# tum-vision/mem

Hardware: AMD Instinct MI355X
Metric: pretrain samples/sec (ViT-B, 224^2 event voxels) (higher is better)
Workload: dtype bf16

## Files before the change

### include/memhip.h

```cpp
#ifndef MEMHIP_H
#define MEMHIP_H

#include <stddef.h>
#include <stdint.h>

#ifdef __cplusplus
extern "C" {
#endif

#define MEMHIP_ABI_VERSION 10

#define MEMHIP_OK 0
#define MEMHIP_EINVAL (-1)
#define MEMHIP_EWORKSPACE (-2)
#define MEMHIP_ELAUNCH (-3)
#define MEMHIP_EUNSUPPORTED (-4)

typedef void* memhip_stream_t;

int memhip_abi_version(void);
const char* memhip_last_error(void);
const char* memhip_arch(void);
const char* memhip_build_flags(void);
int memhip_set_option(const char* name, int value);
// ... 238 lines not shown
  const int32_t* out_map;
  const memhip_dropout_t* dropout;
} memhip_branch_t;
typedef struct memhip_branch_bwd_args {
  const float* dx; int64_t lddx;
  int32_t M, D;
  memhip_branch_t branch;
} memhip_branch_bwd_args_t;
int memhip_branch_bwd(const memhip_branch_bwd_args_t* args, memhip_stream_t stream);
typedef struct memhip_ln_bwd_branch_args {
  const void* dy; int64_t lddy;
  const float* x; int64_t ldx;
  int32_t R, D;
  const float* gamma; const float* mean; const float* rstd;
  float* dres; int64_t lddres;
  float* dgamma; float* dbeta;
  const int32_t* in_map;
  memhip_branch_t branch;
} memhip_ln_bwd_branch_args_t;
int memhip_layernorm_bwd_branch(const memhip_ln_bwd_branch_args_t* args, memhip_stream_t stream);

int memhip_embed_bwd(const float* dx, int64_t lddx, const uint8_t* mask, int B, int L, int D,
                     void* dy_bf16, int64_t lddy, float* dcls, float* dmask_token, memhip_stream_t stream);

int memhip_cross_entropy(void* logits_bf16, int64_t ld, const int64_t* labels, int M, int V,
                         float grad_scale, float* row_loss, int32_t* row_correct, int write_grad,
                         float* out2, memhip_stream_t stream);

int memhip_attn_tokens_padded(int T);
int memhip_relpos_gather(const float* table, const int32_t* index , int T, int TP, int heads,
                         float* bias_pad, float* biasT_pad ,
                         memhip_stream_t stream);
int memhip_attn_fwd(const void* qkv, int64_t ldqkv, int B, int T, int D, int heads, const float* table,
                    int window_h, int window_w, void* out, int64_t ldo, float* lse, memhip_stream_t stream);
int memhip_attn_delta(const void* dout, const void* out, int64_t ldo, int64_t rows, int heads, float* delta,
                      memhip_stream_t stream);
typedef struct memhip_attn_bwd_args {
  const void* qkv; int64_t ldqkv;
  const void* dout; int64_t ldo;
  const void* out; int64_t ldout;
  const float* lse;
  float* delta;
  const float* table;
  int32_t window_h, window_w, B, T, D, heads;
  float scale;
  int32_t reserved0;
  void* dqkv; int64_t lddqkv;
  float* dtable; float* dq_bias; float* dv_bias;
  void* ws; int64_t ws_bytes;
} memhip_attn_bwd_args_t;
// ... 232 lines not shown
```

### mem_amd/csrc/rowops.hip

```cpp
#include "common.h"
#include "dropout.hpp"

#include <type_traits>

namespace {

using namespace memhip;

typedef __attribute__((ext_vector_type(4))) __bf16 bf16x4;
typedef __attribute__((ext_vector_type(8))) __bf16 bf16x8;

__device__ __forceinline__ float wsum(float v) {
  for (int o = 32; o > 0; o >>= 1) v += __shfl_xor(v, o);
  return v;
}
__device__ __forceinline__ float wmax(float v) {
  for (int o = 32; o > 0; o >>= 1) v = fmaxf(v, __shfl_xor(v, o));
  return v;
}

__device__ __forceinline__ float div_newton(float a, float b, float r) {
  const float q0 = a * r;
  return fmaf(fmaf(-q0, b, a), r, q0);
}

constexpr int kMaxChunks = 8;

template <bool FULL>
__device__ __forceinline__ bool chunk_ok(int i, int nch) {
  if constexpr (FULL) return true;
  else return i < nch;
}

// ... 601 lines not shown
        if (k < K) {
          const bf16x4 w = *reinterpret_cast<const bf16x4*>(wr + k);
          const float4 g = *reinterpret_cast<const float4*>(gr + k);
          s[c] += (float)w[0] * g.x + (float)w[1] * g.y + (float)w[2] * g.z + (float)w[3] * g.w;
        }
      }
    }
  }
#pragma unroll
  for (int c = 0; c < 4; ++c) {
    const float t = wsum(s[c]);
    if (lane == 0) red[wave][c] = t;
  }
  __syncthreads();
  if (threadIdx.x < 4 && n0 + (int)threadIdx.x < N) {
    const int n = n0 + threadIdx.x;
    float t = (red[0][threadIdx.x] + red[1][threadIdx.x]) + (red[2][threadIdx.x] + red[3][threadIdx.x]);
    if (b && db) t += b[n] * db[n];
    const float g = gamma[n];
    dgamma[n] = g != 0.f ? t / g : 0.f;
  }
}

__global__ __launch_bounds__(256) void embed_bwd_kernel(const float* __restrict__ dx, long long lddx,
                                                        const unsigned char* __restrict__ mask, int B,
                                                        int L, int D, __bf16* __restrict__ dy,
                                                        long long lddy, float* __restrict__ dcls,
                                                        float* __restrict__ dmask) {
  constexpr int U = 7;
  for (int c = threadIdx.x * 4; c < D; c += 256 * 4) {
    float4 cls{0, 0, 0, 0}, am{0, 0, 0, 0};
    for (int b = blockIdx.x; b < B; b += gridDim.x) {
      const float* row0 = dx + (long long)b * (L + 1) * lddx + c;
      const float4 dc = *reinterpret_cast<const float4*>(row0);
      cls.x += dc.x; cls.y += dc.y; cls.z += dc.z; cls.w += dc.w;
      const unsigned char* mk = mask + (long long)b * L;
      __bf16* out = dy + (long long)b * L * lddy + c;
      int p = 0;
      for (; p + U <= L; p += U) {
        float4 d[U];
#pragma unroll
        for (int u = 0; u < U; ++u) d[u] = *reinterpret_cast<const float4*>(row0 + (long long)(1 + p + u) * lddx);
#pragma unroll
        for (int u = 0; u < U; ++u) {
          const float w = (float)mk[p + u], q = 1.0f - w;
          am.x += d[u].x * w; am.y += d[u].y * w; am.z += d[u].z * w; am.w += d[u].w * w;
          bf16x4 o;
          o[0] = (__bf16)(d[u].x * q); o[1] = (__bf16)(d[u].y * q); o[2] = (__bf16)(d[u].z * q); o[3] = (__bf16)(d[u].w * q);
          *reinterpret_cast<bf16x4*>(out + (long long)(p + u) * lddy) = o;
        }
      }
      for (; p < L; ++p) {
        const float4 d = *reinterpret_cast<const float4*>(row0 + (long long)(1 + p) * lddx);
        const float w = (float)mk[p], q = 1.0f - w;
        am.x += d.x * w; am.y += d.y * w; am.z += d.z * w; am.w += d.w * w;
        bf16x4 o;
        o[0] = (__bf16)(d.x * q); o[1] = (__bf16)(d.y * q); o[2] = (__bf16)(d.z * q); o[3] = (__bf16)(d.w * q);
        *reinterpret_cast<bf16x4*>(out + (long long)p * lddy) = o;
      }
    }
    atomicAdd(dcls + c, cls.x); atomicAdd(dcls + c + 1, cls.y);
    atomicAdd(dcls + c + 2, cls.z); atomicAdd(dcls + c + 3, cls.w);
    atomicAdd(dmask + c, am.x); atomicAdd(dmask + c + 1, am.y);
    atomicAdd(dmask + c + 2, am.z); atomicAdd(dmask + c + 3, am.w);
  }
}

template <int VPT>
__global__ __launch_bounds__(256) void ce_kernel(__bf16* __restrict__ logits, long long ld,
                                                 const long long* __restrict__ labels, int V,
                                                 float grad_scale, float* __restrict__ row_loss,
                                                 int* __restrict__ row_correct, int write_grad) {
  __shared__ float sm[4];
  __shared__ int si[4];
  __shared__ float bc[2];
  const int r = blockIdx.x, tid = threadIdx.x, lane = tid & 63, wave = tid >> 6;
  bf16x8* row = reinterpret_cast<bf16x8*>(logits + (long long)r * ld);
  const int nch = V >> 3;
  float v[VPT][8];
  float mx = -INFINITY;
  int amax = 0x7fffffff;
#pragma unroll
  for (int c = 0; c < VPT; ++c) {
    const int i = tid + c * 256;
    if (i < nch) {
      const bf16x8 t = row[i];
#pragma unroll
// ... 57 lines not shown
        }
        row[i] = o;
      }
    }
  }
}

__global__ __launch_bounds__(256) void ce_reduce_kernel(const float* __restrict__ row_loss,
                                                        const int* __restrict__ row_correct, int M,
                                                        float* __restrict__ out) {
  __shared__ double sd[4];
  __shared__ int sc[4];
  double s = 0.0;
  int c = 0;
  for (int i = threadIdx.x; i < M; i += 256) { s += (double)row_loss[i]; c += row_correct[i]; }
  for (int o = 32; o > 0; o >>= 1) { s += __shfl_xor(s, o); c += __shfl_xor(c, o); }
  if ((threadIdx.x & 63) == 0) { sd[threadIdx.x >> 6] = s; sc[threadIdx.x >> 6] = c; }
  __syncthreads();
  if (threadIdx.x == 0) {
    const double t = (sd[0] + sd[1]) + (sd[2] + sd[3]);
    const int k = sc[0] + sc[1] + sc[2] + sc[3];
    out[0] = (float)(t / (double)M);
    out[1] = (float)k / (float)M;
  }
}

}

template <int MAXN, class F>
void dispatch_width(int D, F&& f) {
  const int nch = cdiv(D / 4, 64);
  const bool full = D % 256 == 0;
  const auto either = [&](auto N) { if (full) f(N, std::true_type{}); else f(N, std::false_type{}); };
  if (nch <= 1) either(std::integral_constant<int, 1>{});
  else if (nch <= 2) either(std::integral_constant<int, 2>{});
  else if (nch <= 3) either(std::integral_constant<int, 3>{});
  else if (MAXN == 4 || nch <= 4) either(std::integral_constant<int, 4>{});
  else if constexpr (MAXN == 8) {
    if (nch == 5 && full) f(std::integral_constant<int, 5>{}, std::true_type{});
    else if (nch == 8 && full) f(std::integral_constant<int, 8>{}, std::true_type{});
    else f(std::integral_constant<int, 8>{}, std::false_type{});
  }
}

extern "C" int memhip_layernorm_fwd(const float* x, int64_t ldx, const int32_t* row_idx, int R, int D,
                                    const float* gamma, const float* beta, float eps, void* y,
// ... 50 lines not shown
  if (M == 0) return MEMHIP_OK;
  MEMHIP_REQUIRE(args->dx && b.dy, "branch_bwd: null pointer");
  MEMHIP_REQUIRE(b.y || !b.dgamma, "branch_bwd: dgamma needs y (or use memhip_layerscale_grad)");
  MEMHIP_REQUIRE(args->lddx % 4 == 0 && b.ldy % 4 == 0 && b.lddy % 4 == 0, "branch_bwd: ld must be a multiple of 4");
  MEMHIP_REQUIRE(D <= 64 * 4 * kBrMaxChunks, "branch_bwd: D=%d too large", D);
  int grid = cdiv(M, 4);
  if (grid > 1024) grid = 1024;
  dispatch_width<kBrMaxChunks>(D, [&](auto N, auto F) {
    dispatch_bool(b.y, [&](auto Y) {
      if (b.dropout) branch_bwd_launch<decltype(N)::value, decltype(F)::value, decltype(Y)::value>(*args, grid, stream, drop_params(*b.dropout));
      else branch_bwd_launch<decltype(N)::value, decltype(F)::value, decltype(Y)::value>(*args, grid, stream);
      return 0;
    });
  });
  return check_launch("branch_bwd");
}

extern "C" int memhip_embed_bwd(const float* dx, int64_t lddx, const uint8_t* mask, int B, int L, int D,
                                void* dy, int64_t lddy, float* dcls, float* dmask_token,
                                memhip_stream_t stream) {
  MEMHIP_REQUIRE(B >= 0 && L > 0 && D > 0 && D % 4 == 0, "embed_bwd: bad shape");
  if (B == 0) return MEMHIP_OK;
  MEMHIP_REQUIRE(dx && mask && dy && dcls && dmask_token, "embed_bwd: null pointer");
  hipLaunchKernelGGL(embed_bwd_kernel, dim3(B < 128 ? B : 128), dim3(256), 0, as_stream(stream), dx, (long long)lddx, mask, B,
                     L, D, (__bf16*)dy, (long long)lddy, dcls, dmask_token);
  return check_launch("embed_bwd");
}

extern "C" int memhip_cross_entropy(void* logits, int64_t ld, const int64_t* labels, int M, int V,
                                    float grad_scale, float* row_loss, int32_t* row_correct,
                                    int write_grad, float* out2, memhip_stream_t stream) {
  MEMHIP_REQUIRE(M >= 0 && V > 0 && V % 8 == 0 && V <= 256 * 8 * 8, "cross_entropy: V=%d unsupported", V);
  if (M == 0) return MEMHIP_OK;
  MEMHIP_REQUIRE(logits && labels && row_loss && row_correct && out2, "cross_entropy: null pointer");
  MEMHIP_REQUIRE(ld % 8 == 0, "cross_entropy: ld must be a multiple of 8");
  hipStream_t s = as_stream(stream);
  const int nch = V / 8, vpt = cdiv(nch, 256);
  __bf16* lg = (__bf16*)logits;
  const long long* lab = (const long long*)labels;
#define CE_LAUNCH(N) hipLaunchKernelGGL(ce_kernel<N>, dim3(M), dim3(256), 0, s, lg, (long long)ld, lab, V, \
                                        grad_scale, row_loss, row_correct, write_grad)
  if (vpt <= 1) CE_LAUNCH(1);
  else if (vpt <= 2) CE_LAUNCH(2);
  else if (vpt <= 4) CE_LAUNCH(4);
  else CE_LAUNCH(8);
#undef CE_LAUNCH
  hipLaunchKernelGGL(ce_reduce_kernel, dim3(1), dim3(256), 0, s, row_loss, row_correct, M, out2);
  return check_launch("cross_entropy");
}

template <int NCH, bool FULL, bool HAS_Y, class... Drop>
static void ln_bwd_branch_launch(const memhip_ln_bwd_branch_args_t& a, int grid, memhip_stream_t stream, Drop... drop) {
  const memhip_branch_t& b = a.branch;
  hipLaunchKernelGGL((ln_bwd_branch_kernel<NCH, FULL, HAS_Y, Drop...>), dim3(grid), dim3(256), (size_t)16 * a.D * sizeof(float),
                     as_stream(stream), (const __bf16*)a.dy, (long long)a.lddy, a.x, (long long)a.ldx, a.R, a.D, a.gamma, a.mean,
                     a.rstd, a.dres, (long long)a.lddres, a.dgamma, a.dbeta, (const __bf16*)b.y, (long long)b.ldy, b.gamma,
                     b.rowmask, b.keep_prob, b.rows_per_sample > 0 ? b.rows_per_sample : 1, (__bf16*)b.dy, (long long)b.lddy,
                     b.dgamma, b.dbias, (const int*)a.in_map, (const int*)b.out_map, drop...);
}

extern "C" int memhip_layernorm_bwd_branch(const memhip_ln_bwd_branch_args_t* args, memhip_stream_t stream) {
  MEMHIP_REQUIRE(args, "layernorm_bwd_branch: null args");
  const memhip_ln_bwd_branch_args_t& a = *args;
  const memhip_branch_t& b = a.branch;
  const int R = a.R, D = a.D;
  MEMHIP_REQUIRE(R >= 0 && D > 0 && D % 4 == 0 && D <= 64 * 4 * 4, "layernorm_bwd_branch: D=%d unsupported (<= 1024)", D);
  MEMHIP_REQUIRE(!b.dropout || D % 8 == 0, "layernorm_bwd_branch_drop: D=%d must be a multiple of 8", D);
  MEMHIP_REQUIRE(!(a.in_map || b.out_map) || (!b.rowmask && !b.y && b.rows_per_sample > 0),
                 "layernorm_bwd_branch: sample maps exclude rowmask / y_branch");
  if (R == 0) return MEMHIP_OK;
  MEMHIP_REQUIRE(a.dy && a.x && a.gamma && a.mean && a.rstd && a.dres && a.dgamma && a.dbeta && b.dy,
// ... 34 lines not shown
```

### mem_amd/ops.py

```python
import ctypes as C

import torch

from ._lib import check, declare, f32, f64, i32, i64, lib, ptr, stream_ptr, sz, vp
from .vae_model import pack_convt_weight

EPI_BIAS_BF16, EPI_BIAS_GELU, EPI_RESIDUAL, EPI_DGELU, EPI_F32, EPI_PATCH_EMBED, EPI_BIAS_GELU_DG, EPI_MUL_AUX = range(8)
EPI_RESIDUAL_DROP = 8


class Dropout(C.Structure):
    _fields_ = [("key0", C.c_uint32), ("key1", C.c_uint32), ("site", C.c_uint32), ("thr", C.c_uint32), ("scale", f32),
                ("row0", i32)]


def dropout_params(key0, key1, site, p, row0=0):
    assert 0.0 <= p < 1.0, p
    return Dropout(int(key0) & 0xFFFFFFFF, int(key1) & 0xFFFFFFFF, int(site), int(round(p * 65536)), 1.0 / (1.0 - p), int(row0))


def with_row0(d, row0):
    return None if d is None else Dropout(d.key0, d.key1, d.site, d.thr, d.scale, int(row0))


# ... 260 lines not shown
        out = torch.empty((M,), dtype=torch.float32, device=logits.device)
    assert out.dtype == torch.float32 and out.numel() >= M
    check(lib.memhip_kl_uniform_rows(ptr(logits), _CONV_MODE[logits.dtype], logits.stride(0), M, N, ptr(out), stream_ptr()),
          "kl_uniform_rows")
    return out[:M]


def tok_flag_samples(gap, rms, B, hw, kappa, lst, count, stats=None):
    check(lib.memhip_tok_flag_samples(ptr(gap), ptr(rms), B, hw, float(kappa), ptr(lst), ptr(count), ptr(stats), stream_ptr()),
          "tok_flag_samples")


def tok_gather_images(x, mean, std, lst, count, offset, R, out, n_round):
    _, Cc, H, W = x.shape
    check(lib.memhip_tok_gather_images_f32(ptr(x), Cc, H, W, ptr(mean), ptr(std), ptr(lst), ptr(count), offset, R, ptr(out),
                                           ptr(n_round), stream_ptr()), "tok_gather_images_f32")


def tok_scatter_ids(ids_in, lst, n_round, offset, R, hw, ids_out):
    check(lib.memhip_tok_scatter_ids(ptr(ids_in), ptr(lst), ptr(n_round), offset, R, hw, ptr(ids_out), stream_ptr()),
          "tok_scatter_ids")


def embed_bwd(dx, mask_u8, B, L, D, dy, dcls, dmask_token):
    check(lib.memhip_embed_bwd(ptr(dx), dx.stride(0), ptr(mask_u8), B, L, D, ptr(dy), dy.stride(0), ptr(dcls),
                               ptr(dmask_token), stream_ptr()), "embed_bwd")


def cross_entropy(logits, labels, M, V, grad_scale, row_loss, row_correct, out2, write_grad=True):
    check(lib.memhip_cross_entropy(ptr(logits), logits.stride(0), ptr(labels), M, V, grad_scale, ptr(row_loss),
                                   ptr(row_correct), int(write_grad), ptr(out2), stream_ptr()), "cross_entropy")


def attn_tokens_padded(T):
    return lib.memhip_attn_tokens_padded(T)


def relpos_gather(table, index_i32, T, TP, heads, bias_pad, biasT_pad=None):
    check(lib.memhip_relpos_gather(ptr(table), ptr(index_i32), T, TP, heads, ptr(bias_pad), ptr(biasT_pad),
                                   stream_ptr()), "relpos_gather")


def attn_fwd(qkv, B, T, D, heads, table, window, out, lse):
    _timed(200, 4.0 * B * T * T * D, lambda: check(
        lib.memhip_attn_fwd(ptr(qkv), qkv.stride(0), B, T, D, heads, ptr(table), window[0], window[1], ptr(out),
                            out.stride(0), ptr(lse), stream_ptr()), "attn_fwd"))


def attn_delta(dout, out, rows, heads, delta):
    check(lib.memhip_attn_delta(ptr(dout), ptr(out), out.stride(0), rows, heads, ptr(delta), stream_ptr()),
          "attn_delta")


def attn_bwd_workspace(B, T, heads, window):
# ... 637 lines not shown
```

### mem_amd/vit_engine.py

```python
import math
from collections import namedtuple

import torch

from . import ops

ALIGN = 1024

Branch = namedtuple("Branch", "n rows gemm_rows ridx smap cmap rowmask keep_prob")


def _pad(n, a):
    return (n + a - 1) // a * a


def flat_layout(shapes, skip, order, aliases=()):
    decays = lambda n: not (len(shapes[n]) == 1 or n.endswith(".bias") or n in skip)
    segs, buckets, flags, off = {}, [], [], 0
    for bname, entries in order:
        b0 = off
        for e in entries:
            if isinstance(e, tuple):
                (n, k), flag = e, 0
            elif e in shapes:
# ... 197 lines not shown
        ops.zero_(self.flat_g[o:o + _pad(k, ALIGN)])

    def set_gelu_dg(self, on):
        self.epi_gelu, self.epi_dgelu = (ops.EPI_BIAS_GELU_DG, ops.EPI_MUL_AUX) if on else (ops.EPI_BIAS_GELU, ops.EPI_DGELU)

    def ensure_batch(self, B, Mm_max, keep=True):
        if B > self.B:
            self._alloc_forward(B)
        if keep and self.B_stash < self.B:
            self._alloc_stash()
        if Mm_max > self.Mm_cap or (self.head_kind == "mlm" and not hasattr(self, "hN")):
            self._alloc_head(min(self.B * self.L, _pad(Mm_max + Mm_max // 16 + 1, 256)))

    def _alloc_head(self, Mm_cap):
        dev, bf, f32 = self.dev, torch.bfloat16, torch.float32
        D, V = self.D, self.V
        e = lambda *s, dt=bf: torch.empty(s, dtype=dt, device=dev)
        if self.head_kind == "mlm":
            self.hN = e(Mm_cap, D)
            self.meanN, self.rstdN = e(Mm_cap, dt=f32), e(Mm_cap, dt=f32)
            self.logits = e(Mm_cap, V)
            self.row_loss, self.row_ok = e(Mm_cap, dt=f32), torch.empty(Mm_cap, dtype=torch.int32, device=dev)
            self.dhN = e(Mm_cap, D)
            self.x_tail, self.dxc = e(max(Mm_cap, 1), D, dt=f32), e(max(Mm_cap, 1), D, dt=f32)
            self.y_tail = torch.zeros((_pad(max(Mm_cap, 1), 256), D), dtype=bf, device=dev)
        self.Mm_cap = Mm_cap

    def _act_set(self, B):
        dev, bf, f32 = self.dev, torch.bfloat16, torch.float32
        D, Hd, M = self.D, self.hidden, B * self.T
        Ma = M + 256
        e = lambda *s, dt=bf: torch.empty(s, dtype=dt, device=dev)
        z = lambda *s, dt=bf: torch.zeros(s, dtype=dt, device=dev)
        return dict(h1=z(Ma, D), qkv=z(Ma, 3 * D), ao=z(Ma, D), h2=z(Ma, D), hpre=z(Ma, Hd),
                    a=z(Ma, Hd), lse=e(B, self.heads, self.TP, dt=f32),
                    mean1=e(M, dt=f32), rstd1=e(M, dt=f32), mean2=e(M, dt=f32), rstd2=e(M, dt=f32))

    def _alloc_forward(self, B):
        dev, f32 = self.dev, torch.float32
        D, T = self.D, self.T
        M = B * T
        self.patches = torch.empty((B * self.L, self.Kpe), dtype=torch.bfloat16, device=dev)
        self.x = [torch.zeros((M + T, D), dtype=f32, device=dev) for _ in range(3)]
        self.act = [self._act_set(B)]
        if self.head_kind != "mlm":
            self.zero_mask = torch.zeros(B * self.L, dtype=torch.uint8, device=dev)
# ... 137 lines not shown

    def _drop(self, site, row0=0):
        key = self.cur["drop_key"] if self.cur else None
        if key is None:
            return None
        return ops.dropout_params(key[0], key[1], site, self.drop_rate, row0)

    def _copy_dropped(self, plan, j, src, dst, B):
        nd = B - plan["n"][j]
        if nd > 0:
            ops.copy_samples(src, dst, plan["drop"][j], nd, self.T * self.D)

    def forward(self, x, mask_u8, rows_idx, labels=None, dp_masks=None, all_tokens=False, labels_event=None):
        assert x.is_cuda and x.dtype == torch.float32 and x.is_contiguous()
        B = x.shape[0]
        assert tuple(x.shape[1:]) == (self.C, self.H, self.W), \
            f"Input image size ({x.shape[2]}*{x.shape[3]}) doesn't match model ({self.H}*{self.W})."
        Mm = rows_idx.numel()
        self.ensure_batch(B, Mm)
        use_tail = (self.tail_rows and not all_tokens and self.depth >= 1 and 0 < Mm and 4 * Mm <= 3 * B * self.T)
        xl = self.forward_trunk(x, mask_u8, dp_masks, tail_rows=rows_idx if use_tail else None)
        D, Hd, T, L, V = self.D, self.hidden, self.T, self.L, self.V
        M = B * T
        self.cur.update(Mm=Mm, rows=rows_idx, labels=labels)
        self._wait_params("head")
        if self.cur.get("tail") is not None:
            ops.layernorm_fwd(self.x_tail, self.P("norm.weight"), self.P("norm.bias"), self.hN, self.meanN, self.rstdN, Mm, D)
        else:
            ops.layernorm_fwd(xl, self.P("norm.weight"), self.P("norm.bias"), self.hN, self.meanN, self.rstdN, Mm, D,
                              row_idx=rows_idx)
        ops.gemm_nt(self.hN, self.W16("lm_head.weight", V, D), Mm, V, D, ops.EPI_BIAS_BF16, out0=self.logits,
                    bias=self.P("lm_head.bias"))
        if labels is not None:
            if labels_event is not None:
                torch.cuda.current_stream().wait_event(labels_event)
            ops.cross_entropy(self.logits, labels, Mm, V, 1.0 / Mm, self.row_loss, self.row_ok, self.loss_acc,
                              write_grad=True)
        return self.logits[:Mm]

    def _split_point(self, B, num_cu=256):
        ntn = max(1, self.D // 256)
        tile_rows = -(-B * self.T // 256)
        rounds = tile_rows * ntn // num_cu
        if rounds < 1:
            return 0
        bs = (rounds * num_cu // ntn) * 256 // self.T
        return bs if 0 < bs < B and (B - bs) * self.T >= 4096 else 0

    def _branch(self, j, b0, b1):
        br = self.cur["branch"][j]
        if b0 == 0 and b1 == self.cur["B"]:
            return br
        assert br.smap is None, "stochastic-depth work skipping runs the whole batch on one stream"
        rows = (b1 - b0) * self.T
        return br._replace(n=b1 - b0, rows=rows, gemm_rows=rows, rowmask=None if br.rowmask is None else br.rowmask[b0:b1])

    def _block_fwd(self, i, b0, b1):
        D, Hd, T = self.D, self.hidden, self.T
        r0, r1 = b0 * T, b1 * T
        pre = f"blocks.{i}."
# ... 226 lines not shown
            return
        e = self._event()
        e.record(self._side)
        torch.cuda.current_stream().wait_event(e)

    def _bucket_ready(self, k):
        if not self.grad_hook:
            return
        if not self._use_side:
            self.grad_hook(k)
            return
        if not self.hook_on_side:
            self._side_join()
            self.grad_hook(k)
            return
        e = self._event()
        e.record()
        with torch.cuda.stream(self._side):
            self._side.wait_event(e)
            self.grad_hook(k)

    attn_ds_workspace = True

    def _attn_ws(self, nb):
        if not self.attn_ds_workspace:
            return None
        need = ops.attn_bwd_workspace(nb, self.T, self.heads, self.window)
        if need == 0:
            return None
        ws = getattr(self, "_attn_ws_buf", None)
        if ws is None or ws.numel() < need:
            ws = self._attn_ws_buf = torch.empty(ops.attn_bwd_workspace(self.cur["B"], self.T, self.heads, self.window),
                                                 dtype=torch.uint8, device=self.dev)
        return ws

    def backward(self, dlogits=None):
        c = self.cur
        B, M, Mm = c["B"], c["M"], c["Mm"]
        D, Hd, T, L, V = self.D, self.hidden, self.T, self.L, self.V
        dp_masks = c["dp"]
        self.wait_optimizer()
        if dlogits is not None:
            self.logits[:Mm].copy_(dlogits)
        if not self.accumulate_grads:
            self._zero_small_grads()
        dx = self.dx
        ops.zero_(dx[:M])
        dl = self.logits
        self._side_begin()
        ops.gemm_nt(dl, self.wT_lm, Mm, D, V, ops.EPI_BIAS_BF16, out0=self.dhN)
        self._on_side(lambda: self._wgrad(dl, self.hN, Mm, V, D, "lm_head.weight", bias_grads=((self.G("lm_head.bias"), 0, V),)))
        if c.get("tail") is not None:
            ops.layernorm_bwd(self.dhN, self.x_tail, self.P("norm.weight"), self.meanN, self.rstdN, self.dxc,
                              self.G("norm.weight"), self.G("norm.bias"), Mm, D, accumulate=False)
            ops.scatter_rows(self.dxc, c["rows"], Mm, D, dx)
        else:
            ops.layernorm_bwd(self.dhN, self.x[2 * self.depth], self.P("norm.weight"), self.meanN, self.rstdN, dx,
                              self.G("norm.weight"), self.G("norm.bias"), Mm, D, accumulate=False, row_idx=c["rows"])
        self._backward_trunk()

    def backward_trunk(self, dxl, dmaps=None):
        c = self.cur
        if not c.get("keep", True):
            raise RuntimeError("backward_trunk after forward_trunk(keep=False): a forward-only pass keeps no activations "
                               "(the blocks shared one buffer set); run the forward with keep=True to train the trunk")
        M, D = c["M"], self.D
        if not self.accumulate_grads:
            self._zero_small_grads(self.head_end)
        if dxl is None:
            ops.zero_(self.dx[:M])
        else:
            self.dx[:M].copy_(dxl.reshape(M, D))
        if dmaps is not None:
            B, n = c["B"], c["B"] * D * self.L
# ... 133 lines not shown
                                         self.G(pre + "norm1.weight"), self.G(pre + "norm1.bias"), M, D, None,
                                         self.P(pb + "gamma_2") if (pb + "gamma_2") in self.segs else None, dY, None,
                                         self.G(pb + "mlp.fc2.bias"), rowmask=bb.rowmask, keep_prob=bb.keep_prob,
                                         rows_per_sample=T, in_map=ba.cmap, out_map=bb.cmap, dropout=self._drop(2 * i - 1))
            elif ba.n > 0:
                ops.layernorm_bwd(self.dh_small, xin, self.P(pre + "norm1.weight"), a["mean1"], a["rstd1"], dx,
                                  self.G(pre + "norm1.weight"), self.G(pre + "norm1.bias"), ba.rows, D, accumulate=True,
                                  row_idx=ba.ridx)
            self._bucket_ready(self.depth - i)
        self._backward_embed(c, B, M)

    def _backward_embed(self, c, B, M):
        D, T, L = self.D, self.T, self.L
        dx = self.dx
        dpos = self._drop(2 * self.depth)
        if dpos is not None:
            ops.dropout_rows(dpos, dx, M, D)
        if self.has_pos:
            if self.accumulate_grads:
                self.G("pos_embed").view(T, D).add_(dx[:M].view(B, T, D).sum(0))
            else:
                self.G("pos_embed").view(T, D).copy_(dx[:M].view(B, T, D).sum(0))
        ops.embed_bwd(dx, c["mask"], B, L, D, self.dYpe, self.G("cls_token"),
                      self.G("mask_token") if "mask_token" in self.segs else self.zero_vec)
        self._on_side(lambda: self._wgrad(self.dYpe, self.patches, B * L, D, self.Kpe, "patch_embed.proj.weight",
                                          bias_grads=((self.G("patch_embed.proj.bias"), 0, D),)))
        self._side_join()
        if self.grad_hook:
            self.grad_hook(self.depth + 1)

    def grad_norm(self, end=None):
        n = self.nflat if end is None else end
        ops.grad_norm(self.flat_g[:n], n, self.gnorm, self.gn_ws)
        return self.gnorm

    def weights_updated(self, end=None):
        if end is None or end >= self.nflat:
            self.weights_dirty = True
        elif not self.weights_dirty:
            assert end <= self.head_end, "partial weight update: the head bucket only (no transposed copies to refresh)"
            ops.cast_f32_bf16(self.flat_p[:end], self.flat_w16[:end], end)
            self.w16_version += 1

    def adamw_step(self, m, v, lr, wd, step, betas=(0.9, 0.95), eps=1e-8, max_norm=0.0):
        if not (self.overlap_optimizer and self.head_kind == "mlm" and not self.fwd_two_streams):
            self.wait_optimizer()
            ops.adamw(self.flat_p, self.flat_g, m, v, self.nflat, self.wd_flags, lr, betas[0], betas[1], eps, wd, step,
                      gnorm=self.gnorm, max_norm=max_norm or 0.0)
            self.weights_dirty = True
# ... 40 lines not shown
```

Baseline: 7633.

## Fuse bias-gradient reductions into cross-entropy and embed backward kernels

Adds a multi-row-per-workgroup cross-entropy kernel that prefetches the next row, accumulates per-workgroup column sums of dlogits in LDS for the lm_head bias gradient, and reduces loss and accuracy in the same launch using a last-block counter. A separate fold kernel sums the partials into the bias gradient on the side stream. The patch-embed bias gradient is likewise accumulated inside embed_bwd. Together these remove the bias reductions from the wgrad GEMMs and drop the separate CE reduce launch, at the cost of an extra workspace, LDS use and more atomics.

```diff
diff --git a/include/memhip.h b/include/memhip.h
--- a/include/memhip.h
+++ b/include/memhip.h
@@ -284,10 +284,39 @@
 
 int memhip_embed_bwd(const float* dx, int64_t lddx, const uint8_t* mask, int B, int L, int D,
                      void* dy_bf16, int64_t lddy, float* dcls, float* dmask_token, memhip_stream_t stream);
+struct memhip_embed_bwd_args {
+  const float* dx; int64_t lddx;
+  const uint8_t* mask;
+  int32_t B, L, D;
+  void* dy; int64_t lddy;
+  float* dcls; float* dmask_token;
+  float* dbias;
+};
+typedef struct memhip_embed_bwd_args memhip_embed_bwd_args_t;
+int memhip_embed_bwd_bias(const memhip_embed_bwd_args_t* args, memhip_stream_t stream);
 
 int memhip_cross_entropy(void* logits_bf16, int64_t ld, const int64_t* labels, int M, int V,
                          float grad_scale, float* row_loss, int32_t* row_correct, int write_grad,
                          float* out2, memhip_stream_t stream);
+struct memhip_ce_args {
+  void* logits; int64_t ld;
+  const int64_t* labels;
+  int32_t M, V;
+  float grad_scale;
+  int32_t write_grad;
+  float* row_loss;
+  int32_t* row_correct;
+  float* out2;
+  int32_t want_bias;
+  int32_t reserved0;
+  float* dbias;
+  void* workspace; size_t workspace_bytes;
+};
+typedef struct memhip_ce_args memhip_ce_args_t;
+int memhip_ce_rows_per_workgroup(int M);
+size_t memhip_ce_workspace(int M, int V);
+int memhip_ce_fused(const memhip_ce_args_t* args, memhip_stream_t stream);
+int memhip_ce_bias_fold(const memhip_ce_args_t* args, memhip_stream_t stream);
 
 int memhip_attn_tokens_padded(int T);
 int memhip_relpos_gather(const float* table, const int32_t* index , int T, int TP, int heads,
diff --git a/mem_amd/csrc/rowops.hip b/mem_amd/csrc/rowops.hip
--- a/mem_amd/csrc/rowops.hip
+++ b/mem_amd/csrc/rowops.hip
@@ -9,6 +9,7 @@
 
 typedef __attribute__((ext_vector_type(4))) __bf16 bf16x4;
 typedef __attribute__((ext_vector_type(8))) __bf16 bf16x8;
+typedef __attribute__((ext_vector_type(4))) unsigned u32x4;
 
 __device__ __forceinline__ float wsum(float v) {
   for (int o = 32; o > 0; o >>= 1) v += __shfl_xor(v, o);
@@ -656,14 +657,15 @@
   }
 }
 
+template <bool BIAS>
 __global__ __launch_bounds__(256) void embed_bwd_kernel(const float* __restrict__ dx, long long lddx,
                                                         const unsigned char* __restrict__ mask, int B,
                                                         int L, int D, __bf16* __restrict__ dy,
                                                         long long lddy, float* __restrict__ dcls,
-                                                        float* __restrict__ dmask) {
+                                                        float* __restrict__ dmask, float* __restrict__ dbias) {
   constexpr int U = 7;
   for (int c = threadIdx.x * 4; c < D; c += 256 * 4) {
-    float4 cls{0, 0, 0, 0}, am{0, 0, 0, 0};
+    float4 cls{0, 0, 0, 0}, am{0, 0, 0, 0}, bs{0, 0, 0, 0};
     for (int b = blockIdx.x; b < B; b += gridDim.x) {
       const float* row0 = dx + (long long)b * (L + 1) * lddx + c;
       const float4 dc = *reinterpret_cast<const float4*>(row0);
@@ -675,6 +677,7 @@
         float4 d[U];
 #pragma unroll
         for (int u = 0; u < U; ++u) d[u] = *reinterpret_cast<const float4*>(row0 + (long long)(1 + p + u) * lddx);
+        float4 t{0, 0, 0, 0};
 #pragma unroll
         for (int u = 0; u < U; ++u) {
           const float w = (float)mk[p + u], q = 1.0f - w;
@@ -682,7 +685,9 @@
           bf16x4 o;
           o[0] = (__bf16)(d[u].x * q); o[1] = (__bf16)(d[u].y * q); o[2] = (__bf16)(d[u].z * q); o[3] = (__bf16)(d[u].w * q);
           *reinterpret_cast<bf16x4*>(out + (long long)(p + u) * lddy) = o;
-        }
+          if constexpr (BIAS) { t.x += (float)o[0]; t.y += (float)o[1]; t.z += (float)o[2]; t.w += (float)o[3]; }
+        }
+        if constexpr (BIAS) { bs.x += t.x; bs.y += t.y; bs.z += t.z; bs.w += t.w; }
       }
       for (; p < L; ++p) {
         const float4 d = *reinterpret_cast<const float4*>(row0 + (long long)(1 + p) * lddx);
@@ -691,12 +696,17 @@
         bf16x4 o;
         o[0] = (__bf16)(d.x * q); o[1] = (__bf16)(d.y * q); o[2] = (__bf16)(d.z * q); o[3] = (__bf16)(d.w * q);
         *reinterpret_cast<bf16x4*>(out + (long long)p * lddy) = o;
+        if constexpr (BIAS) { bs.x += (float)o[0]; bs.y += (float)o[1]; bs.z += (float)o[2]; bs.w += (float)o[3]; }
       }
     }
     atomicAdd(dcls + c, cls.x); atomicAdd(dcls + c + 1, cls.y);
     atomicAdd(dcls + c + 2, cls.z); atomicAdd(dcls + c + 3, cls.w);
     atomicAdd(dmask + c, am.x); atomicAdd(dmask + c + 1, am.y);
     atomicAdd(dmask + c + 2, am.z); atomicAdd(dmask + c + 3, am.w);
+    if constexpr (BIAS) {
+      atomicAdd(dbias + c, bs.x); atomicAdd(dbias + c + 1, bs.y);
+      atomicAdd(dbias + c + 2, bs.z); atomicAdd(dbias + c + 3, bs.w);
+    }
   }
 }
 
@@ -800,6 +810,211 @@
     const int k = sc[0] + sc[1] + sc[2] + sc[3];
     out[0] = (float)(t / (double)M);
     out[1] = (float)k / (float)M;
+  }
+}
+
+constexpr int kCeMaxGrid = 1024, kCeMinRows = 8;
+inline int ce_rows_per_wg(int M) { const int r = cdiv(M, kCeMaxGrid); return r < kCeMinRows ? kCeMinRows : r; }
+struct CeSlot { double loss; int hits; int pad; };
+constexpr size_t kCeSlotOffset = 256;
+constexpr size_t kCePartOffset = kCeSlotOffset + kCeMaxGrid * sizeof(CeSlot);
+
+template <int VPT, bool BIAS, bool FULL>
+__global__ __launch_bounds__(256) __attribute__((amdgpu_waves_per_eu(VPT <= 4 ? 4 : 2))) void ce_rows_kernel(__bf16* __restrict__ logits, long long ld,
+                                                      const long long* __restrict__ labels, int M, int V, int rows_per_wg,
+                                                      float grad_scale, float* __restrict__ row_loss,
+                                                      int* __restrict__ row_correct, int write_grad,
+                                                      unsigned* __restrict__ counter, CeSlot* __restrict__ slots,
+                                                      float* __restrict__ part, float* __restrict__ out2) {
+  __shared__ float sm[4];
+  __shared__ int si[4];
+  __shared__ float bc[3];
+  __shared__ double sd[4];
+  __shared__ int sc[4];
+  __shared__ int last;
+  const int tid = threadIdx.x, lane = tid & 63, wave = tid >> 6;
+  const int nch = V >> 3;
+  const int r0 = blockIdx.x * rows_per_wg, r1 = min(M, r0 + rows_per_wg);
+  extern __shared__ float4 cacc[];
+  if constexpr (BIAS) {
+#pragma unroll
+    for (int c = 0; c < 2 * VPT; ++c) cacc[c * 256 + tid] = float4{0, 0, 0, 0};
+  }
+  double wl = 0.0;
+  int wh = 0;
+  u32x4 nx[VPT];
+  auto issue = [&](int r) {
+    const u32x4* row = reinterpret_cast<const u32x4*>(logits + (long long)r * ld);
+#pragma unroll
+    for (int c = 0; c < VPT; ++c) {
+      const int i = tid + c * 256;
+      if (FULL || i < nch) nx[c] = row[i];
+    }
+  };
+  if (r0 < r1) issue(r0);
+  for (int r = r0; r < r1; ++r) {
+    bf16x8* row = reinterpret_cast<bf16x8*>(logits + (long long)r * ld);
+    const long long lab = labels[r];
+    float v[VPT][8];
+    float mx = -INFINITY;
+    int amax = 0x7fffffff;
+#pragma unroll
+    for (int c = 0; c < VPT; ++c) {
+      const int i = tid + c * 256;
+      if (FULL || i < nch) {
+        const bf16x8 t = __builtin_bit_cast(bf16x8, nx[c]);
+#pragma unroll
+        for (int k = 0; k < 8; ++k) {
+          v[c][k] = (float)t[k];
+          if (v[c][k] > mx) { mx = v[c][k]; amax = i * 8 + k; }
+        }
+      }
+    }
+    if (r + 1 < r1) issue(r + 1);
+    for (int o = 32; o > 0; o >>= 1) {
+      const float om = __shfl_xor(mx, o);
+      const int oi = __shfl_xor(amax, o);
+      if (om > mx || (om == mx && oi < amax)) { mx = om; amax = oi; }
+    }
+    if (lane == 0) { sm[wave] = mx; si[wave] = amax; }
+    __syncthreads();
+    if (tid == 0) {
+      float m = sm[0]; int a = si[0];
+      for (int w = 1; w < 4; ++w) if (sm[w] > m || (sm[w] == m && si[w] < a)) { m = sm[w]; a = si[w]; }
+      bc[0] = m; si[0] = a;
+    }
+    __syncthreads();
+    mx = bc[0];
+    amax = si[0];
+    const bool lab_ok = lab >= 0 && lab < V;
+    const int lchunk = lab_ok ? (int)(lab >> 3) : 0, lk = (int)(lab & 7);
+    if (tid == (lchunk & 255)) {
+      float zl = __builtin_nanf("");
+      if (lab_ok) {
+#pragma unroll
+        for (int c = 0; c < VPT; ++c)
+#pragma unroll
+          for (int k = 0; k < 8; ++k)
+            if (c == (lchunk >> 8) && k == lk) zl = v[c][k];
+      }
+      bc[2] = zl;
+    }
+    float s = 0.f;
+#pragma unroll
+    for (int c = 0; c < VPT; ++c) {
+      const int i = tid + c * 256;
+      if (FULL || i < nch) {
+#pragma unroll
+        for (int k = 0; k < 8; ++k) { v[c][k] = __expf(v[c][k] - mx); s += v[c][k]; }
+      }
+    }
+    s = wsum(s);
+    __syncthreads();
+    if (lane == 0) sm[wave] = s;
+    __syncthreads();
+    if (tid == 0) bc[1] = (sm[0] + sm[1]) + (sm[2] + sm[3]);
+    __syncthreads();
+    const float sum = bc[1];
+#pragma unroll
+    for (int c = 0; c < VPT; ++c) asm volatile("" : "+v"(nx[c]));
+    if (write_grad) {
+      const float inv = 1.0f / sum;
+      const int lown = lab_ok ? lchunk : -1;
+#pragma unroll
+      for (int c = 0; c < VPT; ++c) {
+        const int i = tid + c * 256;
+        if (FULL || i < nch) {
+          bf16x8 o;
+#pragma unroll
+          for (int k = 0; k < 8; ++k) {
+            const bool own = i == lown && k == lk;
+            const float p = own ? __fmaf_rn(v[c][k], inv, -1.0f) : mul_rn(v[c][k], inv);
+            o[k] = (__bf16)mul_rn(p, grad_scale);
+          }
+          row[i] = o;
+          if constexpr (BIAS) {
+            float4 lo = cacc[2 * c * 256 + tid], hi = cacc[(2 * c + 1) * 256 + tid];
+            lo.x += (float)o[0]; lo.y += (float)o[1]; lo.z += (float)o[2]; lo.w += (float)o[3];
+            hi.x += (float)o[4]; hi.y += (float)o[5]; hi.z += (float)o[6]; hi.w += (float)o[7];
+            cacc[2 * c * 256 + tid] = lo; cacc[(2 * c + 1) * 256 + tid] = hi;
+          }
+        }
+      }
+    }
+    if (tid == 0) {
+      const float l = (mx + __logf(sum)) - bc[2];
+      const int hit = (amax == (int)lab) ? 1 : 0;
+      row_loss[r] = l;
+      row_correct[r] = hit;
+      wl += (double)l;
+      wh += hit;
+    }
+  }
+  if constexpr (BIAS) {
+    float4* prow = reinterpret_cast<float4*>(part + (long long)blockIdx.x * V);
+#pragma unroll
+    for (int c = 0; c < VPT; ++c) {
+      const int i = tid + c * 256;
+      if (FULL || i < nch) {
+        prow[2 * i] = cacc[2 * c * 256 + tid];
+        prow[2 * i + 1] = cacc[(2 * c + 1) * 256 + tid];
+      }
+    }
+  }
+  if (tid == 0) {
+    slots[blockIdx.x].loss = wl;
+    slots[blockIdx.x].hits = wh;
+    __threadfence();
+    last = atomicAdd(counter, 1u) == gridDim.x - 1 ? 1 : 0;
+  }
+  __syncthreads();
+  if (!last) return;
+  __threadfence();
+  double t = 0.0;
+  int h = 0;
+  for (int i = tid; i < (int)gridDim.x; i += 256) {
+    t += __longlong_as_double((long long)__hip_atomic_load(reinterpret_cast<unsigned long long*>(&slots[i].loss), __ATOMIC_RELAXED,
+                                                            __HIP_MEMORY_SCOPE_AGENT));
+    h += __hip_atomic_load(&slots[i].hits, __ATOMIC_RELAXED, __HIP_MEMORY_SCOPE_AGENT);
+  }
+  for (int o = 32; o > 0; o >>= 1) { t += __shfl_xor(t, o); h += __shfl_xor(h, o); }
+  if (lane == 0) { sd[wave] = t; sc[wave] = h; }
+  __syncthreads();
+  if (tid == 0) {
+    const double tt = (sd[0] + sd[1]) + (sd[2] + sd[3]);
+    const int k = sc[0] + sc[1] + sc[2] + sc[3];
+    out2[0] = (float)(tt / (double)M);
+    out2[1] = (float)k / (float)M;
+    __hip_atomic_store(counter, 0u, __ATOMIC_RELAXED, __HIP_MEMORY_SCOPE_AGENT);
+  }
+}
+
+__global__ __launch_bounds__(256) void ce_bias_fold_kernel(const float* __restrict__ part, int G, int V, float* __restrict__ dbias) {
+  __shared__ float4 red[16][16];
+  const int tx = threadIdx.x & 15, ty = threadIdx.x >> 4;
+  const int col = blockIdx.x * 64 + tx * 4;
+  float4 s{0, 0, 0, 0};
+  if (col < V) {
+    int g = ty;
+    for (; g + 7 * 16 < G; g += 8 * 16) {
+      float4 t[8];
+#pragma unroll
+      for (int u = 0; u < 8; ++u) t[u] = *reinterpret_cast<const float4*>(part + (long long)(g + u * 16) * V + col);
+#pragma unroll
+      for (int u = 0; u < 8; ++u) { s.x += t[u].x; s.y += t[u].y; s.z += t[u].z; s.w += t[u].w; }
+    }
+    for (; g < G; g += 16) {
+      const float4 t = *reinterpret_cast<const float4*>(part + (long long)g * V + col);
+      s.x += t.x; s.y += t.y; s.z += t.z; s.w += t.w;
+    }
+  }
+  red[ty][tx] = s;
+  __syncthreads();
+  if (ty == 0 && col < V) {
+    float4 t = red[0][tx];
+    for (int g = 1; g < 16; ++g) { t.x += red[g][tx].x; t.y += red[g][tx].y; t.z += red[g][tx].z; t.w += red[g][tx].w; }
+    float* o = dbias + col;
+    o[0] += t.x; o[1] += t.y; o[2] += t.z; o[3] += t.w;
   }
 }
 
@@ -896,9 +1111,21 @@
   MEMHIP_REQUIRE(B >= 0 && L > 0 && D > 0 && D % 4 == 0, "embed_bwd: bad shape");
   if (B == 0) return MEMHIP_OK;
   MEMHIP_REQUIRE(dx && mask && dy && dcls && dmask_token, "embed_bwd: null pointer");
-  hipLaunchKernelGGL(embed_bwd_kernel, dim3(B < 128 ? B : 128), dim3(256), 0, as_stream(stream), dx, (long long)lddx, mask, B,
-                     L, D, (__bf16*)dy, (long long)lddy, dcls, dmask_token);
+  hipLaunchKernelGGL(embed_bwd_kernel<false>, dim3(B < 128 ? B : 128), dim3(256), 0, as_stream(stream), dx, (long long)lddx, mask, B,
+                     L, D, (__bf16*)dy, (long long)lddy, dcls, dmask_token, (float*)nullptr);
   return check_launch("embed_bwd");
+}
+
+extern "C" int memhip_embed_bwd_bias(const memhip_embed_bwd_args_t* args, memhip_stream_t stream) {
+  MEMHIP_REQUIRE(args, "embed_bwd_bias: null args");
+  const memhip_embed_bwd_args_t& a = *args;
+  if (!a.dbias) return memhip_embed_bwd(a.dx, a.lddx, a.mask, a.B, a.L, a.D, a.dy, a.lddy, a.dcls, a.dmask_token, stream);
+  MEMHIP_REQUIRE(a.B >= 0 && a.L > 0 && a.D > 0 && a.D % 4 == 0, "embed_bwd_bias: bad shape");
+  if (a.B == 0) return MEMHIP_OK;
+  MEMHIP_REQUIRE(a.dx && a.mask && a.dy && a.dcls && a.dmask_token, "embed_bwd_bias: null pointer");
+  hipLaunchKernelGGL(embed_bwd_kernel<true>, dim3(a.B < 128 ? a.B : 128), dim3(256), 0, as_stream(stream), a.dx, (long long)a.lddx,
+                     a.mask, a.B, a.L, a.D, (__bf16*)a.dy, (long long)a.lddy, a.dcls, a.dmask_token, a.dbias);
+  return check_launch("embed_bwd_bias");
 }
 
 extern "C" int memhip_cross_entropy(void* logits, int64_t ld, const int64_t* labels, int M, int V,
@@ -921,6 +1148,71 @@
 #undef CE_LAUNCH
   hipLaunchKernelGGL(ce_reduce_kernel, dim3(1), dim3(256), 0, s, row_loss, row_correct, M, out2);
   return check_launch("cross_entropy");
+}
+
+extern "C" int memhip_ce_rows_per_workgroup(int M) { return ce_rows_per_wg(M > 0 ? M : 1); }
+
+extern "C" size_t memhip_ce_workspace(int M, int V) {
+  if (M <= 0 || V <= 0) return 0;
+  return kCePartOffset + (size_t)cdiv(M, ce_rows_per_wg(M)) * (size_t)V * sizeof(float);
+}
+
+static int ce_validate(const memhip_ce_args_t& a, const char* who) {
+  MEMHIP_REQUIRE(a.M >= 0 && a.V > 0 && a.V % 8 == 0 && a.V <= 256 * 8 * 8, "%s: V=%d unsupported", who, a.V);
+  if (a.M == 0) return MEMHIP_OK;
+  MEMHIP_REQUIRE(a.workspace && ((uintptr_t)a.workspace & 15) == 0, "%s: workspace must be 16-byte aligned", who);
+  if (a.workspace_bytes < memhip_ce_workspace(a.M, a.V))
+    return fail(MEMHIP_EWORKSPACE, "%s: workspace %zu < %zu bytes", who, a.workspace_bytes, memhip_ce_workspace(a.M, a.V));
+  return MEMHIP_OK;
+}
+
+extern "C" int memhip_ce_fused(const memhip_ce_args_t* args, memhip_stream_t stream) {
+  MEMHIP_REQUIRE(args, "ce_fused: null args");
+  const memhip_ce_args_t& a = *args;
+  if (const int rc = ce_validate(a, "ce_fused")) return rc;
+  if (a.M == 0) return MEMHIP_OK;
+  MEMHIP_REQUIRE(a.logits && a.labels && a.row_loss && a.row_correct && a.out2, "ce_fused: null pointer");
+  MEMHIP_REQUIRE(a.ld % 8 == 0 && ((uintptr_t)a.logits & 15) == 0, "ce_fused: logits must be 16-byte aligned, ld a multiple of 8");
+  MEMHIP_REQUIRE(!a.want_bias || a.write_grad, "ce_fused: want_bias needs write_grad (the sums are those of dlogits)");
+  MEMHIP_REQUIRE(!a.want_bias || a.V <= 256 * 8 * 4, "ce_fused: want_bias serves V <= 8192 (the sums of a workgroup live in 4 * V bytes of LDS), got %d", a.V);
+  const int rows = ce_rows_per_wg(a.M), grid = cdiv(a.M, rows);
+  char* ws = (char*)a.workspace;
+  const int vpt = cdiv(a.V / 8, 256);
+  const auto launch = [&](auto N, auto B) {
+    constexpr int vp = decltype(N)::value;
+    constexpr bool bias = decltype(B)::value;
+    if (a.V == vp * 2048)
+      hipLaunchKernelGGL((ce_rows_kernel<vp, bias, true>), dim3(grid), dim3(256), bias ? (size_t)vp * 2 * 256 * sizeof(float4) : 0, as_stream(stream),
+                         (__bf16*)a.logits, (long long)a.ld, (const long long*)a.labels, a.M, a.V, rows, a.grad_scale, a.row_loss,
+                         (int*)a.row_correct, a.write_grad, (unsigned*)ws, (CeSlot*)(ws + kCeSlotOffset), (float*)(ws + kCePartOffset),
+                         a.out2);
+    else
+      hipLaunchKernelGGL((ce_rows_kernel<vp, bias, false>), dim3(grid), dim3(256), bias ? (size_t)vp * 2 * 256 * sizeof(float4) : 0, as_stream(stream),
+                       (__bf16*)a.logits, (long long)a.ld, (const long long*)a.labels, a.M, a.V, rows, a.grad_scale, a.row_loss,
+                       (int*)a.row_correct, a.write_grad, (unsigned*)ws, (CeSlot*)(ws + kCeSlotOffset), (float*)(ws + kCePartOffset),
+                       a.out2);
+    return 0;
+  };
+  const auto width = [&](auto B) {
+    if (vpt <= 1) launch(std::integral_constant<int, 1>{}, B);
+    else if (vpt <= 2) launch(std::integral_constant<int, 2>{}, B);
+    else if (vpt <= 4) launch(std::integral_constant<int, 4>{}, B);
+    else launch(std::integral_constant<int, 8>{}, B);
+    return 0;
+  };
+  dispatch_bool(a.want_bias != 0, width);
+  return check_launch("ce_fused");
+}
+
+extern "C" int memhip_ce_bias_fold(const memhip_ce_args_t* args, memhip_stream_t stream) {
+  MEMHIP_REQUIRE(args, "ce_bias_fold: null args");
+  const memhip_ce_args_t& a = *args;
+  if (const int rc = ce_validate(a, "ce_bias_fold")) return rc;
+  if (a.M == 0) return MEMHIP_OK;
+  MEMHIP_REQUIRE(a.dbias, "ce_bias_fold: null pointer");
+  hipLaunchKernelGGL(ce_bias_fold_kernel, dim3(cdiv(a.V, 64)), dim3(256), 0, as_stream(stream),
+                     (const float*)((const char*)a.workspace + kCePartOffset), cdiv(a.M, ce_rows_per_wg(a.M)), a.V, a.dbias);
+  return check_launch("ce_bias_fold");
 }
 
 template <int NCH, bool FULL, bool HAS_Y, class... Drop>
diff --git a/mem_amd/ops.py b/mem_amd/ops.py
--- a/mem_amd/ops.py
+++ b/mem_amd/ops.py
@@ -306,14 +306,60 @@
           "tok_scatter_ids")
 
 
-def embed_bwd(dx, mask_u8, B, L, D, dy, dcls, dmask_token):
-    check(lib.memhip_embed_bwd(ptr(dx), dx.stride(0), ptr(mask_u8), B, L, D, ptr(dy), dy.stride(0), ptr(dcls),
-                               ptr(dmask_token), stream_ptr()), "embed_bwd")
+class EmbedBwdArgs(C.Structure):
+    _fields_ = [("dx", vp), ("lddx", i64), ("mask", vp), ("B", i32), ("L", i32), ("D", i32), ("dy", vp), ("lddy", i64),
+                ("dcls", vp), ("dmask_token", vp), ("dbias", vp)]
+
+
+class CeArgs(C.Structure):
+    _fields_ = [("logits", vp), ("ld", i64), ("labels", vp), ("M", i32), ("V", i32), ("grad_scale", f32), ("write_grad", i32),
+                ("row_loss", vp), ("row_correct", vp), ("out2", vp), ("want_bias", i32), ("reserved0", i32), ("dbias", vp),
+                ("workspace", vp), ("workspace_bytes", sz)]
+
+
+declare({"memhip_embed_bwd_bias": (i32, [C.POINTER(EmbedBwdArgs), vp]),
+         "memhip_ce_rows_per_workgroup": (i32, [i32]),
+         "memhip_ce_workspace": (sz, [i32, i32]),
+         "memhip_ce_fused": (i32, [C.POINTER(CeArgs), vp]),
+         "memhip_ce_bias_fold": (i32, [C.POINTER(CeArgs), vp])})
+
+
+def embed_bwd(dx, mask_u8, B, L, D, dy, dcls, dmask_token, dbias=None):
+    if dbias is None:
+        check(lib.memhip_embed_bwd(ptr(dx), dx.stride(0), ptr(mask_u8), B, L, D, ptr(dy), dy.stride(0), ptr(dcls),
+                                   ptr(dmask_token), stream_ptr()), "embed_bwd")
+        return
+    a = EmbedBwdArgs(_p(dx), dx.stride(0), _p(mask_u8), B, L, D, _p(dy), dy.stride(0), _p(dcls), _p(dmask_token), _p(dbias))
+    check(lib.memhip_embed_bwd_bias(C.byref(a), stream_ptr()), "embed_bwd_bias")
 
 
 def cross_entropy(logits, labels, M, V, grad_scale, row_loss, row_correct, out2, write_grad=True):
     check(lib.memhip_cross_entropy(ptr(logits), logits.stride(0), ptr(labels), M, V, grad_scale, ptr(row_loss),
                                    ptr(row_correct), int(write_grad), ptr(out2), stream_ptr()), "cross_entropy")
+
+
+def ce_rows_per_workgroup(M):
+    return lib.memhip_ce_rows_per_workgroup(M)
+
+
+def ce_workspace(M, V):
+    return int(lib.memhip_ce_workspace(M, V))
+
+
+def _ce_args(logits, labels, M, V, grad_scale, row_loss, row_correct, out2, write_grad, want_bias, dbias, workspace):
+    assert workspace.dtype == torch.uint8
+    return CeArgs(_p(logits), 0 if logits is None else logits.stride(0), _p(labels), M, V, grad_scale, int(write_grad),
+                  _p(row_loss), _p(row_correct), _p(out2), int(want_bias), 0, _p(dbias), _p(workspace), workspace.numel())
+
+
+def ce_fused(logits, labels, M, V, grad_scale, row_loss, row_correct, out2, workspace, write_grad=True, want_bias=True):
+    a = _ce_args(logits, labels, M, V, grad_scale, row_loss, row_correct, out2, write_grad, want_bias, None, workspace)
+    check(lib.memhip_ce_fused(C.byref(a), stream_ptr()), "ce_fused")
+
+
+def ce_bias_fold(M, V, workspace, dbias):
+    a = _ce_args(None, None, M, V, 0.0, None, None, None, True, True, dbias, workspace)
+    check(lib.memhip_ce_bias_fold(C.byref(a), stream_ptr()), "ce_bias_fold")
 
 
 def attn_tokens_padded(T):
diff --git a/mem_amd/vit_engine.py b/mem_amd/vit_engine.py
--- a/mem_amd/vit_engine.py
+++ b/mem_amd/vit_engine.py
@@ -243,6 +243,7 @@
             self.logits = e(Mm_cap, V)
             self.row_loss, self.row_ok = e(Mm_cap, dt=f32), torch.empty(Mm_cap, dtype=torch.int32, device=dev)
             self.dhN = e(Mm_cap, D)
+            self.ce_ws = torch.zeros(ops.ce_workspace(max(1, min(Mm_cap, 8192)), V), dtype=torch.uint8, device=dev)
             self.x_tail, self.dxc = e(max(Mm_cap, 1), D, dt=f32), e(max(Mm_cap, 1), D, dt=f32)
             self.y_tail = torch.zeros((_pad(max(Mm_cap, 1), 256), D), dtype=bf, device=dev)
         self.Mm_cap = Mm_cap
@@ -426,7 +427,7 @@
         xl = self.forward_trunk(x, mask_u8, dp_masks, tail_rows=rows_idx if use_tail else None)
         D, Hd, T, L, V = self.D, self.hidden, self.T, self.L, self.V
         M = B * T
-        self.cur.update(Mm=Mm, rows=rows_idx, labels=labels)
+        self.cur.update(Mm=Mm, rows=rows_idx, labels=labels, ce_bias=False)
         self._wait_params("head")
         if self.cur.get("tail") is not None:
             ops.layernorm_fwd(self.x_tail, self.P("norm.weight"), self.P("norm.bias"), self.hN, self.meanN, self.rstdN, Mm, D)
@@ -438,8 +439,13 @@
         if labels is not None:
             if labels_event is not None:
                 torch.cuda.current_stream().wait_event(labels_event)
-            ops.cross_entropy(self.logits, labels, Mm, V, 1.0 / Mm, self.row_loss, self.row_ok, self.loss_acc,
-                              write_grad=True)
+            if self.fused_ce and V <= 8192:
+                ops.ce_fused(self.logits, labels, Mm, V, 1.0 / Mm, self.row_loss, self.row_ok, self.loss_acc, self.ce_ws,
+                             write_grad=True, want_bias=True)
+                self.cur["ce_bias"] = True
+            else:
+                ops.cross_entropy(self.logits, labels, Mm, V, 1.0 / Mm, self.row_loss, self.row_ok, self.loss_acc,
+                                  write_grad=True)
         return self.logits[:Mm]
 
     def _split_point(self, B, num_cu=256):
@@ -712,6 +718,8 @@
 
     attn_ds_workspace = True
 
+    fused_ce = True
+
     def _attn_ws(self, nb):
         if not self.attn_ds_workspace:
             return None
@@ -739,7 +747,13 @@
         dl = self.logits
         self._side_begin()
         ops.gemm_nt(dl, self.wT_lm, Mm, D, V, ops.EPI_BIAS_BF16, out0=self.dhN)
-        self._on_side(lambda: self._wgrad(dl, self.hN, Mm, V, D, "lm_head.weight", bias_grads=((self.G("lm_head.bias"), 0, V),)))
+        if dlogits is None and c.get("ce_bias"):
+            def head_wgrad():
+                self._wgrad(dl, self.hN, Mm, V, D, "lm_head.weight")
+                ops.ce_bias_fold(Mm, V, self.ce_ws, self.G("lm_head.bias"))
+            self._on_side(head_wgrad)
+        else:
+            self._on_side(lambda: self._wgrad(dl, self.hN, Mm, V, D, "lm_head.weight", bias_grads=((self.G("lm_head.bias"), 0, V),)))
         if c.get("tail") is not None:
             ops.layernorm_bwd(self.dhN, self.x_tail, self.P("norm.weight"), self.meanN, self.rstdN, self.dxc,
                               self.G("norm.weight"), self.G("norm.bias"), Mm, D, accumulate=False)
@@ -919,9 +933,9 @@
             else:
                 self.G("pos_embed").view(T, D).copy_(dx[:M].view(B, T, D).sum(0))
         ops.embed_bwd(dx, c["mask"], B, L, D, self.dYpe, self.G("cls_token"),
-                      self.G("mask_token") if "mask_token" in self.segs else self.zero_vec)
-        self._on_side(lambda: self._wgrad(self.dYpe, self.patches, B * L, D, self.Kpe, "patch_embed.proj.weight",
-                                          bias_grads=((self.G("patch_embed.proj.bias"), 0, D),)))
+                      self.G("mask_token") if "mask_token" in self.segs else self.zero_vec,
+                      dbias=self.G("patch_embed.proj.bias"))
+        self._on_side(lambda: self._wgrad(self.dYpe, self.patches, B * L, D, self.Kpe, "patch_embed.proj.weight"))
         self._side_join()
         if self.grad_hook:
             self.grad_hook(self.depth + 1)
```

After: 7620. No clear change (-0.2%).
